# trzy/FasterRCNN

Measured on AMD Instinct MI355X. Metric: images/sec (600x1000) Faster-RCNN VGG-16 inference, higher is better.
Workload: dtype f32 (float32 tensors and accumulation; 15 GEMM layers in the f32x3 split-operand emulation = two fp16 terms per block-scaled operand, three fp16 MFMAs per product; 0 in f32x6 = three bf16 terms, six bf16 MFMAs; the other 2 on exact-f32 MFMA; strict exact-f32 everywhere: config.strict_f32_images_per_

## Files before the change

fasterrcnn_amd/_native.py:

```python
import ctypes as C
import os

_HERE = os.path.dirname(os.path.abspath(__file__))
LIB_PATH = os.environ.get("FRCNN_LIB_PATH") or os.path.join(_HERE, "csrc", "libfrcnn_hip.so")

OK = 0
ABI_VERSION = 21
ERRORS = {0: "FRCNN_OK", -1: "FRCNN_EINVAL", -2: "FRCNN_EHIP", -3: "FRCNN_ENOMEM",
          -4: "FRCNN_EUNSUPPORTED", -5: "FRCNN_ENODEVICE"}
RELU = 1
POOL2 = 2
NUM_KCLASS = 11
KCLASS_NAMES = ("conv3x3_mfma", "conv3x3_c3", "linear_mfma", "proposals", "roi_pool", "other", "winograd_transforms",
                "winograd_gemm", "winograd_x6_transforms", "winograd_x6_gemm", "winograd_x3f")

SYMBOLS = (
    "frcnn_abi_version", "frcnn_error_string", "frcnn_last_hip_error", "frcnn_device_count",
    "frcnn_anchors", "frcnn_pack_conv3x3", "frcnn_pack_conv3x3_c3", "frcnn_pack_fc_chw_to_hwc",
    "frcnn_pack_stack_rows", "frcnn_conv3x3_c3", "frcnn_conv3x3_c3_cmax", "frcnn_conv3x3_workspace_bytes", "frcnn_conv3x3_nhwc",
    "frcnn_maxpool2x2_nhwc",
    "frcnn_linear_workspace_bytes", "frcnn_linear", "frcnn_softmax_rows", "frcnn_rpn_proposals",
    "frcnn_nms", "frcnn_roi_pool", "frcnn_roi_pool_x3t", "frcnn_detections", "frcnn_ctx_create", "frcnn_ctx_create_proposals", "frcnn_ctx_destroy",
    "frcnn_ctx_bytes", "frcnn_vgg16_forward", "frcnn_ctx_tensor", "frcnn_ctx_timing_enable",
    "frcnn_ctx_timing_read",
    "frcnn_output_block_layout", "frcnn_stream_depend", "frcnn_ctx_submit_stats", "frcnn_predict_submit", "frcnn_streams_share_queue",
    "frcnn_fold_bn_pack", "frcnn_conv_workspace_bytes", "frcnn_conv_nhwc", "frcnn_conv_nhwc_math", "frcnn_conv_nhwc_x3g", "frcnn_conv_nhwc_x3g_tickets", "frcnn_pack_conv_x3g_weights", "frcnn_x3_saturation_events", "frcnn_tensor_absmax", "frcnn_conv7x7_s2_c3",
    "frcnn_maxpool3x3_s2_nhwc", "frcnn_spatial_mean_nhwc", "frcnn_resnet_forward", "frcnn_rpn_targets",
    "frcnn_preprocess_workspace_bytes", "frcnn_preprocess",
    "frcnn_conv3x3_uses_winograd", "frcnn_resnet_block_uses_winograd", "frcnn_pack_conv3x3_winograd",
    "frcnn_pack_conv3x3_winograd_taps", "frcnn_conv3x3_winograd_workspace_bytes",
    "frcnn_conv3x3_nhwc_winograd",
    "frcnn_conv3x3_uses_winograd_fused", "frcnn_resnet_block_uses_winograd_fused", "frcnn_pack_conv3x3_winograd_fused", "frcnn_pack_conv3x3_winograd_fused_taps",
    "frcnn_conv3x3_nhwc_winograd_fused",
    "frcnn_roi_align", "frcnn_roi_align_backward",
    "frcnn_x6t_record_bytes", "frcnn_split_rows_x6t", "frcnn_gemm_x6t_workspace_bytes", "frcnn_gemm_x6t", "frcnn_split_pixels_x6t", "frcnn_split_patches3x3_x6t",
    "frcnn_conv3x3_uses_winograd_x6", "frcnn_conv3x3_winograd_x6_pack_bytes", "frcnn_pack_conv3x3_winograd_x6",
    "frcnn_conv3x3_winograd_x6_workspace_bytes", "frcnn_conv3x3_nhwc_winograd_x6",
    "frcnn_pixel_absmax", "frcnn_split_pixels_x3t", "frcnn_split_patches3x3_x3t",
    "frcnn_x3t_blob_bytes", "frcnn_pack_rows_x3t", "frcnn_conv3x3_winograd_x3_pack_bytes", "frcnn_pack_conv3x3_winograd_x3",
    "frcnn_conv3x3_winograd_x3_workspace_bytes", "frcnn_conv3x3_nhwc_winograd_x3",
    "frcnn_conv3x3_winograd_x3_fused_workspace_bytes", "frcnn_conv3x3_nhwc_winograd_x3_fused", "frcnn_conv3x3_nhwc_winograd_x3_chain",
    "frcnn_x3t_record_bytes", "frcnn_rows_scale_x3t", "frcnn_split_rows_x3t", "frcnn_gemm_x3t_workspace_bytes", "frcnn_gemm_x3t",
    "frcnn_conv3x3_nhwc_winograd_fused_maps", "frcnn_ctx_create_backbone", "frcnn_resnet_backbone", "frcnn_resnet_forward_features", "frcnn_resnet_rpn_roipool", "frcnn_ctx_create_head", "frcnn_resnet_head",
    "frcnn_label_proposals", "frcnn_gather_rows", "frcnn_rpn_loss", "frcnn_detector_loss",
    "frcnn_gemm_tn_math", "frcnn_conv3x3_wgrad_math", "frcnn_conv_wgrad_math", "frcnn_bottleneck_backward_workspace_bytes", "frcnn_bottleneck_backward",
    "frcnn_gemm_tn_workspace_bytes", "frcnn_gemm_tn", "frcnn_conv3x3_wgrad_workspace_bytes", "frcnn_conv3x3_wgrad",
    "frcnn_pack_conv3x3_dgrad", "frcnn_relu_backward", "frcnn_dropout", "frcnn_dropout_relu_backward", "frcnn_add_inplace", "frcnn_maxpool2x2_backward",
    "frcnn_roi_pool_backward_workspace_bytes", "frcnn_roi_pool_backward", "frcnn_transpose", "frcnn_sgd_step", "frcnn_sgd_step_fold",
    "frcnn_conv_wgrad_workspace_bytes", "frcnn_conv_wgrad", "frcnn_conv_dgrad_workspace_bytes", "frcnn_conv_dgrad", "frcnn_conv_dgrad_math",
    "frcnn_pack_conv_dgrad", "frcnn_scale_rows", "frcnn_bn_scale_shift", "frcnn_spatial_mean_backward",
    "frcnn_ops_roi_align", "frcnn_ops_roi_align_backward", "frcnn_ops_roi_pool", "frcnn_ops_roi_pool_backward",
    "frcnn_ops_nms_workspace_bytes", "frcnn_ops_nms",
    "frcnn_ops_ms_roi_align", "frcnn_ops_ms_roi_align_workspace_bytes", "frcnn_ops_ms_roi_align_backward",
    "frcnn_ops_half_run", "frcnn_ops_roi_align_16", "frcnn_ops_roi_align_backward_16", "frcnn_ops_roi_pool_16",
    "frcnn_ops_roi_pool_backward_16", "frcnn_ops_ms_roi_align_16", "frcnn_ops_ms_roi_align_backward_16",
    "frcnn_ops_ps_roi_pool", "frcnn_ops_ps_roi_pool_backward", "frcnn_ops_ps_roi_align", "frcnn_ops_ps_roi_align_backward",
    "frcnn_ops_ps_roi_pool_16", "frcnn_ops_ps_roi_pool_backward_16", "frcnn_ops_ps_roi_align_16", "frcnn_ops_ps_roi_align_backward_16",
    "frcnn_ops_deform_workspace_bytes", "frcnn_ops_deform_forward", "frcnn_ops_deform_backward_columns", "frcnn_ops_deform_backward_offset",
    "frcnn_ops_deform_input_plan", "frcnn_ops_deform_backward_input", "frcnn_ops_deform_backward_weight",
    "frcnn_ops_deform_workspace_bytes_16", "frcnn_ops_deform_forward_16", "frcnn_ops_deform_backward_columns_16",
    "frcnn_ops_deform_backward_offset_16", "frcnn_ops_deform_input_plan_16", "frcnn_ops_deform_backward_input_16",
    "frcnn_ops_deform_backward_weight_16",
    "frcnn_ops_deform_roi_pool_cull_list", "frcnn_ops_deform_roi_pool_workspace_bytes", "frcnn_ops_deform_roi_pool",
    "frcnn_ops_deform_roi_pool_backward", "frcnn_ops_deform_roi_pool_16", "frcnn_ops_deform_roi_pool_backward_16",
    "frcnn_ops_box_iou_rotated", "frcnn_ops_nms_rotated", "frcnn_ops_roi_align_rotated_cull_list", "frcnn_ops_roi_align_rotated",
# ... 349 lines not shown
    "frcnn_maxpool3x3_s2_nhwc": (C.c_int, [_vp, _vp, _i, _i, _i, _vp]),
    "frcnn_spatial_mean_nhwc": (C.c_int, [_vp, _vp, _i, _i, _i, _i, _vp]),
    "frcnn_resnet_forward": (C.c_int, [_vp, C.POINTER(ResNetWeights), C.POINTER(ForwardParams), _vp, _i, _i,
                                       _vp, _vp, _vp, _vp, _vp, _vp, _vp]),
    "frcnn_resnet_forward_features": (C.c_int, [_vp, C.POINTER(ResNetWeights), C.POINTER(ForwardParams), _vp, _i, _i,
                                                _vp, _vp, _vp, _vp, _vp, _vp, _vp]),
    "frcnn_resnet_backbone": (C.c_int, [_vp, C.POINTER(ResNetWeights), C.POINTER(ForwardParams), _vp, _i, _i, _i, _vp, _vp]),
    "frcnn_pixel_absmax": (C.c_int, [_vp, _vp, C.c_longlong, _i, _vp]),
    "frcnn_split_pixels_x3t": (C.c_int, [_vp, _vp, _vp, _vp, _i, _i, _i, _i, _i, _i, _vp]),
    "frcnn_split_patches3x3_x3t": (C.c_int, [_vp, _vp, _vp, _vp, _i, _i, _i, _i, _i, _i, _vp]),
    "frcnn_x3t_blob_bytes": (C.c_size_t, [_i, _i, _i]),
    "frcnn_pack_rows_x3t": (C.c_int, [_vp, _i, _sz, _vp, _i, _i, _i, _i, _vp]),
    "frcnn_conv3x3_winograd_x3_pack_bytes": (C.c_size_t, [_i, _i]),
    "frcnn_pack_conv3x3_winograd_x3": (C.c_int, [_vp, _vp, _i, _i, _vp]),
    "frcnn_conv3x3_winograd_x3_workspace_bytes": (C.c_size_t, [_i, _i, _i, _i, _i]),
    "frcnn_conv3x3_nhwc_winograd_x3": (C.c_int, [_vp, _vp, _vp, _vp, _i, _i, _i, _i, _i, _u, _vp, _sz, _vp]),
    "frcnn_conv3x3_winograd_x3_fused_workspace_bytes": (C.c_size_t, [_i, _i, _i]),
    "frcnn_conv3x3_nhwc_winograd_x3_fused": (C.c_int, [_vp, _vp, _vp, _vp, _i, _i, _i, _i, _i, _u, _vp, _sz, _vp]),
    "frcnn_conv3x3_nhwc_winograd_x3_chain": (C.c_int, [_vp, _vp, _vp, _vp, _i, _i, _i, _i, _i, _u, _i, _vp, _sz, _vp, _vp, _vp]),
    "frcnn_x3t_record_bytes": (C.c_size_t, [_i, _i]),
    "frcnn_rows_scale_x3t": (C.c_int, [_vp, _i, _sz, _vp, _i, _i, _i, _i, _vp]),
    "frcnn_split_rows_x3t": (C.c_int, [_vp, _i, _sz, _vp, _vp, _i, _i, _i, _i, _vp]),
    "frcnn_gemm_x3t_workspace_bytes": (C.c_size_t, [_i, _i, _i, _i]),
    "frcnn_gemm_x3t": (C.c_int, [_vp, _vp, _i, _sz, _sz, _vp, _vp, _i, _sz, _sz, _vp, _vp, _vp, _i, _sz, _i, _i, _i, _i, _u, _vp, _sz, _vp]),
    "frcnn_ctx_create_backbone": (C.c_int, [C.POINTER(C.c_void_p), _i, _i, _i]),
    "frcnn_ctx_create_head": (C.c_int, [C.POINTER(C.c_void_p), _i]),
    "frcnn_resnet_rpn_roipool": (C.c_int, [_vp, C.POINTER(ResNetWeights), C.POINTER(ForwardParams), _vp, _i, _i, _vp, _vp, _vp, _vp, _vp, _vp]),
    "frcnn_resnet_head": (C.c_int, [_vp, C.POINTER(ResNetWeights), C.POINTER(ForwardParams), _vp, _i, _vp, _vp, _vp]),
    "frcnn_conv3x3_nhwc_winograd_fused_maps": (C.c_int, [_vp, _vp, _vp, _vp, _i, _i, _i, _i, _i, _u, _vp]),
    "frcnn_label_proposals": (C.c_int, [_vp, _vp, _i, _vp, _vp, _i, _i, _f, _f, C.POINTER(C.c_float), C.POINTER(C.c_float),
                                        _vp, _vp, _vp, _vp, _vp, _vp]),
    "frcnn_gather_rows": (C.c_int, [_vp, _vp, _i, _i, _vp, _vp]),
    "frcnn_rpn_loss": (C.c_int, [_vp, _i, _i, _vp, _i, _vp, _vp, _vp, _vp]),
    "frcnn_detector_loss": (C.c_int, [_vp, _vp, _vp, _vp, _i, _i, _vp, _vp, _i, _vp]),
    "frcnn_gemm_tn_workspace_bytes": (C.c_size_t, [_i, _i, _i]),
    "frcnn_gemm_tn": (C.c_int, [_vp, _i, _vp, _i, _vp, _i, _i, _i, _i, _vp, _sz, _vp]),
    "frcnn_gemm_tn_math": (C.c_int, [_vp, _i, _vp, _i, _vp, _i, _i, _i, _i, _i, _vp, _sz, _vp]),
    "frcnn_conv3x3_wgrad_math": (C.c_int, [_vp, _vp, _vp, _i, _i, _i, _i, _i, _vp, _sz, _vp]),
    "frcnn_conv_wgrad_math": (C.c_int, [_vp, _vp, _vp, _i, _i, _i, _i, _i, _i, _i, _i, _i, _vp, _sz, _vp]),
    "frcnn_bottleneck_backward_workspace_bytes": (C.c_int, [_vp, _vp, _vp, _vp, _i, _i, _i, _i, _i, C.POINTER(C.c_size_t), C.POINTER(C.c_size_t)]),
    "frcnn_bottleneck_backward": (C.c_int, [_vp, _vp, _vp, _vp, _vp, _vp, _vp, _vp, _vp, _vp, _vp, _vp, _vp, _i, _i, _i, _i, _i, _i, _vp, _sz, _vp, _sz,
                                            _vp, _vp]),
    "frcnn_conv3x3_wgrad_workspace_bytes": (C.c_size_t, [_i, _i, _i, _i]),
    "frcnn_conv3x3_wgrad": (C.c_int, [_vp, _vp, _vp, _i, _i, _i, _i, _vp, _sz, _vp]),
    "frcnn_pack_conv3x3_dgrad": (C.c_int, [_vp, _vp, _i, _i, _vp]),
    "frcnn_conv_wgrad_workspace_bytes": (C.c_size_t, [_i] * 8),
# ... 96 lines not shown
```

fasterrcnn_amd/csrc/api.hip:

```cpp
#include "common.h"
#include <algorithm>
#include <cmath>
#include <cstring>
#include <initializer_list>
#include <string>
#include <vector>
#include <new>

namespace frcnn {

static thread_local std::string g_hip_error;
void set_hip_error(hipError_t e) { g_hip_error = hipGetErrorString(e); }

static size_t align_up(size_t v, size_t a) { return (v + a - 1) / a * a; }

struct EventRec { int cls; hipEvent_t start, stop; };

struct Scratch {
    void* p = nullptr;
    size_t bytes = 0;
    int reserve(size_t want, hipStream_t s, bool zero)
    {
        if (want <= bytes) return FRCNN_OK;
        if (p) { FRCNN_HIP_TRY(hipStreamSynchronize(s)); release(); }
// ... 308 lines not shown
    if (!d_a || !d_inv_scale) return FRCNN_EINVAL;
    return launch_rows_scale_x3t(d_a, lda, a_batch_floats, d_inv_scale, rows, rows_padded, K, batches, as_stream(stream));
}

int frcnn_split_rows_x3t(const float* d_a, int lda, size_t a_batch_floats, const float* d_inv_scale, void* d_rec, int rows, int rows_padded,
                         int K, int batches, void* stream)
{
    if (!d_a || !d_rec || !d_inv_scale) return FRCNN_EINVAL;
    return launch_split_rows_x3t(d_a, lda, a_batch_floats, d_inv_scale, d_rec, rows, rows_padded, K, batches, as_stream(stream));
}

size_t frcnn_gemm_x3t_workspace_bytes(int M, int N, int K, int batches) { return gemm_x3t_workspace_bytes(M, N, K, batches); }

int frcnn_gemm_x3t(const void* d_a_rec, const float* d_a_inv, int a_rows, size_t a_batch_bytes, size_t a_inv_batch_floats,
                   const void* d_b_rec, const float* d_b_inv, int b_rows, size_t b_batch_bytes, size_t b_inv_batch_floats,
                   const float* d_bias, const float* d_residual, float* d_c, int ldc, size_t c_batch_floats, int M, int N, int K,
                   int batches, unsigned flags, void* d_ws, size_t ws_bytes, void* stream)
{
    return launch_gemm_x3t(d_a_rec, d_a_inv, a_rows, a_batch_bytes, a_inv_batch_floats, d_b_rec, d_b_inv, b_rows, b_batch_bytes,
                           b_inv_batch_floats, d_bias, d_residual, d_c, ldc, c_batch_floats, M, N, K, batches, flags, d_ws, ws_bytes,
                           as_stream(stream));
}

size_t frcnn_conv3x3_winograd_x3_fused_workspace_bytes(int n_maps, int H, int W)
{
    return n_maps > 0 && H > 0 && W > 0 ? conv3x3_winograd_x3_fused_workspace_bytes(n_maps, H, W) : 0;
}

int frcnn_conv3x3_nhwc_winograd_x3_fused(const float* d_x, const void* d_blob, const float* d_bias, float* d_y, int n_maps, int H, int W,
                                         int cin, int cout, unsigned flags, void* d_ws, size_t ws_bytes, void* stream)
{
    if (!d_x || !d_blob || !d_bias || !d_y) return FRCNN_EINVAL;
    return launch_conv3x3_winograd_x3_fused(d_x, d_blob, d_bias, d_y, n_maps, H, W, cin, cout, flags, d_ws, ws_bytes, as_stream(stream));
}

int frcnn_pixel_absmax(const float* d_x, float* d_cmax, long long pixels, int c, void* stream)
{
    if (!d_x || !d_cmax) return FRCNN_EINVAL;
    return launch_pixel_absmax(d_x, d_cmax, pixels, c, as_stream(stream));
}

int frcnn_split_pixels_x3t(const float* d_x, const float* d_cmax, void* d_rec, float* d_inv_scale, int n_maps, int H, int W, int c, int stride,
                           int rows_padded, void* stream)
{
    if (!d_x || !d_rec) return FRCNN_EINVAL;
    return launch_split_pixels_x3t(d_x, d_cmax, d_rec, d_inv_scale, n_maps, H, W, c, stride, rows_padded, as_stream(stream));
// ... 1582 lines not shown
```

fasterrcnn_amd/csrc/common.h:

```cpp
#pragma once
#include <hip/hip_runtime.h>
#include <stdint.h>
#include <stddef.h>
#include <stdlib.h>
#include "../../include/frcnn_hip.h"

typedef float f32x4  __attribute__((ext_vector_type(4)));
typedef float f32x16 __attribute__((ext_vector_type(16)));

inline const char* frcnn_knob(const char* name)
{
#ifdef FRCNN_EXPERIMENT_KNOBS
    return getenv(name);
#else
    (void)name;
    return nullptr;
#endif
}

namespace frcnn {

void set_hip_error(hipError_t e);

inline int check_launch() {
// ... 108 lines not shown
size_t gemm_x6t_workspace_bytes(int M, int N, int K, int batches);
void gemm_x6t_set_tiles(int mode);
int launch_gemm_x6t(const void* a_rec, int a_rows, size_t a_batch_bytes, const void* b_rec, int b_rows, size_t b_batch_bytes,
                    const float* bias, const float* residual, float* c, int ldc, size_t c_batch_floats, int M, int N, int K, int batches,
                    unsigned flags, void* ws, size_t ws_bytes, hipStream_t s, int tiles_mode = -1);
int launch_split_pixels_x6t(const float* x, void* rec, int N, int H, int W, int C, int stride, int rows_padded, hipStream_t s);
int gemm_x6t_get_tiles();
int launch_gemm_x6t_reduce(const float* ws, const float* bias, const float* residual, float* c, int ldc, size_t c_batch_floats, int M, int N,
                           int batches, int splits, int relu, hipStream_t s);
size_t x3t_record_bytes(int rows_padded, int K);
int launch_rows_scale_x3t(const float* a, int lda, size_t a_batch_floats, float* inv_scale, int R, int rows_padded, int K, int batches,
                          hipStream_t s);
int launch_split_rows_x3t(const float* a, int lda, size_t a_batch_floats, const float* inv_scale, void* rec, int R, int rows_padded, int K,
                          int batches, hipStream_t s);
int launch_split_pixels_x3t(const float* x, const float* cmax, void* rec, float* inv, int N, int H, int W, int C, int stride, int rows_padded,
                            hipStream_t s);
int launch_split_patches3x3_x3t(const float* x, const float* cmax, void* rec, float* inv, int N, int H, int W, int C, int stride,
                                int rows_padded, hipStream_t s);
size_t gemm_x3t_workspace_bytes(int M, int N, int K, int batches);
int launch_gemm_x3t(const void* a_rec, const float* a_inv, int a_rows, size_t a_batch_bytes, size_t a_inv_batch, const void* b_rec,
                    const float* b_inv, int b_rows, size_t b_batch_bytes, size_t b_inv_batch, const float* bias, const float* residual,
                    float* c, int ldc, size_t c_batch_floats, int M, int N, int K, int batches, unsigned flags, void* ws, size_t ws_bytes,
                    hipStream_t s, int tiles_mode = -1);
size_t x3t_blob_bytes(int rows_padded, int K, int batches);
int launch_pack_rows_x3t(const float* a, int lda, size_t a_batch_floats, void* blob, int R, int rows_padded, int K, int batches, hipStream_t s);
int launch_pixel_absmax(const float* x, float* cmax, long long pixels, int C, hipStream_t s);
size_t conv3x3_winograd_x3_pack_bytes(int cout, int cin);
int launch_pack_conv3x3_winograd_x3(const float* u_f32, void* ublob, int cout, int cin, hipStream_t s);
size_t conv3x3_winograd_x3_workspace_bytes(int N, int H, int W, int cin, int cout);
int winograd_x3_plan(int N, int H, int W, int cin, int cout, unsigned flags, void* ws, size_t ws_bytes, void** V, float** vinv, float** cmax,
                     float** M, void** G, size_t* g_bytes);
int launch_winograd_x3_input(const float* x, float* cmax, void* vrec, float* vinv, int N, int H, int W, int cin, hipStream_t s,
                             const float* cmax_ready = nullptr);
int launch_winograd_x3_gemm(const void* vrec, const float* vinv, const void* ublob, float* M, int N, int H, int W, int cin, int cout, void* gws,
                            size_t gws_bytes, hipStream_t s);
int launch_conv3x3_winograd_x3(const float* x, const void* ublob, const float* b, float* y, int N, int H, int W, int cin, int cout,
                               unsigned flags, void* ws, size_t ws_bytes, hipStream_t s,
                               const float* cmax_ready = nullptr, float* cmax_out = nullptr);
size_t conv3x3_winograd_x3_fused_workspace_bytes(int N, int H, int W);
int launch_conv3x3_winograd_x3_fused(const float* x, const void* ublob, const float* b, float* y, int N, int H, int W, int cin, int cout,
                                     unsigned flags, void* ws, size_t ws_bytes, hipStream_t s, const float* cmax_ready = nullptr,
                                     float* cmax_out = nullptr);
int launch_roi_pool_x3t(const float* fm, int fh, int fw, int c, const float* rois, const int32_t* n_rois, int max_rois, int pooled,
                        float scale, float* cmax, float* inv, void* rec, int rec_rows, hipStream_t s, bool cmax_ready = false);
bool conv3x3_uses_winograd_x6(int cin, int cout);
size_t conv3x3_winograd_x6_pack_bytes(int cout, int cin);
// ... 105 lines not shown
```

fasterrcnn_amd/csrc/gemm_x3t.hip:

```cpp
#include "x3t.h"

namespace frcnn {

typedef _Float16 hx_f16x8 __attribute__((ext_vector_type(8)));

#ifndef HX_ABLATE
#define HX_ABLATE 0
#endif
__global__ __launch_bounds__(256)
void rows_scale_x3t_kernel(const float* __restrict__ a, int lda, size_t a_batch, float* __restrict__ inv_scale, int R, int rows_padded,
                           int K, int batches)
{
    const int lane = threadIdx.x & 63;
    const long long wave = (long long)blockIdx.x * 4 + (threadIdx.x >> 6);
    if (wave >= (long long)batches * rows_padded) return;
    const int row = (int)(wave % rows_padded), batch = (int)(wave / rows_padded);
    float mx = 0.f;
    if (row < R) {
        const float* src = a + (size_t)batch * a_batch + (size_t)row * lda;
        for (int k = 4 * lane; k < K; k += 256) {
            const f32x4 v = *reinterpret_cast<const f32x4*>(src + k);
            mx = fmaxf(fmaxf(mx, fmaxf(fabsf(v[0]), fabsf(v[1]))), fmaxf(fabsf(v[2]), fabsf(v[3])));
        }
    }
#pragma unroll
    for (int off = 32; off >= 1; off >>= 1) mx = fmaxf(mx, __shfl_xor(mx, off));
    float mult, inv;
    hx_row_scale(mx, mult, inv);
// ... 361 lines not shown
                for (int e = 0; e < 4; ++e) v[e] = (acc[i][j][4 * g + e] * sa) * sb[e];
                if (direct && p.bias != nullptr) v = v + *reinterpret_cast<const f32x4*>(p.bias + n);
                if (direct && p.residual != nullptr)
                    v = v + *reinterpret_cast<const f32x4*>(p.residual + (size_t)batch * p.c_batch + (size_t)m * ldd + n);
                if (direct && p.relu) {
#pragma unroll
                    for (int e = 0; e < 4; ++e) v[e] = fmaxf(v[e], 0.f);
                }
                if (HX_ABLATE & 4) asm volatile("" ::"v"(v));
                else *reinterpret_cast<f32x4*>(row + n) = v;
            }
        }
    }
#ifdef HX_CLOCKS
    if (lane == 0 && p.ws != nullptr) {
        const unsigned long long real_exit = __builtin_amdgcn_s_memrealtime();
        float* o = p.ws + ((size_t)blockIdx.x * C::NW + wave) * 8;
        o[0] = (float)(clk1 - clk0); o[1] = (float)(real1 - real0); o[2] = (float)(real0 - real_entry); o[3] = (float)(real_exit - real1);
        o[4] = (float)nst; o[5] = (float)(real_entry & 0xFFFFFF); o[6] = (float)(real_exit & 0xFFFFFF); o[7] = 1.0f;
    }
#endif
}

size_t x3t_record_bytes(int rows_padded, int K) { return (size_t)(K / 16) * (rows_padded / 32) * HX_RB; }

int launch_rows_scale_x3t(const float* a, int lda, size_t a_batch_floats, float* inv_scale, int R, int rows_padded, int K, int batches,
                          hipStream_t s)
{
    if (R < 1 || rows_padded < R || rows_padded % 32 != 0 || K < 16 || K % 16 != 0 || lda < K || lda % 4 != 0 || batches < 1)
        return FRCNN_EINVAL;
    const long long waves = (long long)batches * rows_padded;
    const long long blocks = (waves + 3) / 4;
    if (blocks > 0x7fffffffLL) return FRCNN_EINVAL;
    hipLaunchKernelGGL(rows_scale_x3t_kernel, dim3((unsigned)blocks), dim3(256), 0, s, a, lda, a_batch_floats, inv_scale, R, rows_padded, K,
                       batches);
    return check_launch();
}

int launch_split_rows_x3t(const float* a, int lda, size_t a_batch_floats, const float* inv_scale, void* rec, int R, int rows_padded, int K,
                          int batches, hipStream_t s)
{
    if (R < 1 || rows_padded < R || rows_padded % 32 != 0 || K < 16 || K % 16 != 0 || lda < K || lda % 4 != 0 || batches < 1 || !inv_scale)
        return FRCNN_EINVAL;
    const long long waves = (long long)batches * (K / 16) * (rows_padded / 32);
    const long long blocks = (waves + 3) / 4;
    if (blocks > 0x7fffffffLL) return FRCNN_EINVAL;
// ... 15 lines not shown
        return check_launch();
    }
    const long long waves = (long long)(C / 16) * (rows_padded / 32);
    hipLaunchKernelGGL(split_pixels_x3t_kernel, dim3((unsigned)((waves + 3) / 4)), dim3(256), 0, s, x, cmax, static_cast<unsigned char*>(rec),
                       inv, H, W, Ho, Wo, C, stride, (int)R, rows_padded / 32, C / 16);
    return check_launch();
}

int launch_split_patches3x3_x3t(const float* x, const float* cmax, void* rec, float* inv, int N, int H, int W, int C, int stride,
                                int rows_padded, hipStream_t s)
{
    if (N < 1 || H < 1 || W < 1 || C < 16 || C % 16 != 0 || stride < 1 || stride > 2 || rows_padded % 32 != 0 || !cmax || !inv) return FRCNN_EINVAL;
    const int Ho = (H - 1) / stride + 1, Wo = (W - 1) / stride + 1;
    const long long R = (long long)N * Ho * Wo;
    if (R > rows_padded || R > 0x7fffffffLL) return FRCNN_EINVAL;
    const long long waves = (long long)(9 * C / 16) * (rows_padded / 32);
    hipLaunchKernelGGL(split_patches3x3_x3t_kernel, dim3((unsigned)((waves + 3) / 4)), dim3(256), 0, s, x, cmax,
                       static_cast<unsigned char*>(rec), inv, H, W, Ho, Wo, C, stride, (int)R, rows_padded / 32, 9 * C / 16);
    return check_launch();
}

struct HxPlan { int cfg, mtiles, ntiles, splits, chunks_per_split; };

static HxPlan plan_gemm_x3t(int M, int N, int K, int batches, int tiles_mode = -1)
{
    HxPlan pl;
    const int chunks = K / 16;
    static const int env_force = []() { const char* e = frcnn_knob("FRCNN_HX_CFG"); return e ? atoi(e) : -1; }();
    const int mode = tiles_mode >= 0 ? tiles_mode : gemm_x6t_get_tiles();
    const int force = (env_force >= 0 && tiles_mode < 0) ? env_force : (mode == 1 ? 0 : mode == 2 ? 1 : -1);
    const long long u0 = (long long)cdiv(M, 320) * cdiv(N, 256) * batches;
    const long long u1 = (long long)cdiv(M, 160) * cdiv(N, 128) * batches;
    int splits0 = 1;
    while (u0 * splits0 * 2 <= 256 && chunks / (splits0 * 2) >= 8) splits0 *= 2;
    const double c0 = (double)((u0 * splits0 + 255) / 256) * 1920.0 / splits0 + (splits0 > 1 ? 600.0 : 0.0);
    int splits1 = 1;
    while (u1 * splits1 * 2 <= 256 && chunks / (splits1 * 2) >= 8) splits1 *= 2;
    const double c1 = (double)((u1 * splits1 + 255) / 256) * 480.0 / 0.85 / splits1 + (splits1 > 1 ? 600.0 : 0.0);
    pl.cfg = (force == 0 || force == 1) ? force : (c1 < c0 ? 1 : 0);
    static const bool big_unsplit = frcnn_knob("FRCNN_HX_BIG_UNSPLIT") != nullptr;
    if (big_unsplit && force < 0 && pl.cfg == 1 && splits1 == 1) { pl.cfg = 0; splits0 = 1; }
    int splits = pl.cfg == 1 ? splits1 : splits0;
    if (splits > chunks) splits = chunks;
    pl.mtiles = pl.cfg == 1 ? cdiv(M, 160) : cdiv(M, 320);
    pl.ntiles = pl.cfg == 1 ? cdiv(N, 128) : cdiv(N, 256);
    pl.chunks_per_split = cdiv(chunks, splits);
    pl.splits = cdiv(chunks, pl.chunks_per_split);
    return pl;
}

size_t gemm_x3t_workspace_bytes(int M, int N, int K, int batches)
{
    if (!gemm_x6t_shape_ok(M, N, K, batches)) return 0;
    size_t need = 0;
    for (int mode = 0; mode < 3; ++mode) {
        const HxPlan pl = plan_gemm_x3t(M, N, K, batches, mode);
        const size_t b = pl.splits > 1 ? (size_t)pl.splits * batches * M * N * sizeof(float) : 0;
        if (b > need) need = b;
    }
    return need;
}

int launch_gemm_x3t(const void* a_rec, const float* a_inv, int a_rows, size_t a_batch_bytes, size_t a_inv_batch, const void* b_rec,
                    const float* b_inv, int b_rows, size_t b_batch_bytes, size_t b_inv_batch, const float* bias, const float* residual,
                    float* c, int ldc, size_t c_batch_floats, int M, int N, int K, int batches, unsigned flags, void* ws, size_t ws_bytes,
                    hipStream_t s, int tiles_mode)
{
    if (!gemm_x6t_shape_ok(M, N, K, batches)) return FRCNN_EUNSUPPORTED;
    if (!a_rec || !b_rec || !a_inv || !b_inv || !c || a_rows % 320 != 0 || a_rows < M || b_rows % 256 != 0 || b_rows < N || ldc < N ||
        ldc % 4 != 0)
        return FRCNN_EINVAL;
    const HxPlan pl = plan_gemm_x3t(M, N, K, batches, tiles_mode);
    if (pl.splits > 1 && (ws == nullptr || ws_bytes < (size_t)pl.splits * batches * M * N * sizeof(float))) return FRCNN_EINVAL;
    HxParams p;
    p.a = static_cast<const unsigned char*>(a_rec);
    p.b = static_cast<const unsigned char*>(b_rec);
    p.a_inv = a_inv; p.b_inv = b_inv;
    p.c = c;
    p.ws = static_cast<float*>(ws);
    p.bias = bias;
    p.residual = residual;
    p.a_batch = a_batch_bytes; p.b_batch = b_batch_bytes; p.c_batch = c_batch_floats;
    p.a_inv_batch = a_inv_batch; p.b_inv_batch = b_inv_batch;
    p.a_rbt = a_rows / 32; p.b_rbt = b_rows / 32;
    p.M = M; p.N = N; p.ldc = ldc;
    p.nchunks = K / 16; p.chunks_per_split = pl.chunks_per_split; p.splits = pl.splits; p.batches = batches;
    p.mtiles = pl.mtiles; p.ntiles = pl.ntiles;
    p.relu = (flags & FRCNN_RELU) ? 1 : 0;
    const long long total = (long long)pl.mtiles * pl.ntiles * batches * pl.splits;
    if (total > 0x7fffffffLL) return FRCNN_EINVAL;
    p.total = (int)total;
    static const int env_nsub = []() { const char* e = frcnn_knob("FRCNN_HX_NSUB"); return e ? atoi(e) : 0; }();
    const int last = p.nchunks - (pl.splits - 1) * pl.chunks_per_split;
    const bool even = pl.chunks_per_split % 2 == 0 && last % 2 == 0;
    const int nsub = !even ? 1 : (env_nsub == 1 || env_nsub == 2) ? env_nsub : (pl.chunks_per_split >= 64 ? 2 : 1);
#define HX_LAUNCH(TM, TN, VM, VN, NS)                                                                          \
    do {                                                                                                      \
        using C = HxCfg<TM, TN, VM, VN, NS>;                                                                    \
        auto kern = gemm_x3t_kernel<TM, TN, VM, VN, NS>;                                                        \
        FRCNN_MAX_LDS_ONCE(kern, C::LDS_BYTES);                                                                 \
        hipLaunchKernelGGL(kern, dim3((unsigned)total), dim3(C::THREADS), C::LDS_BYTES, s, p);                  \
    } while (0)
    if (pl.cfg == 1) { if (nsub == 2) HX_LAUNCH(5, 1, 1, 4, 2); else HX_LAUNCH(5, 1, 1, 4, 1); }
    else             { if (nsub == 2) HX_LAUNCH(5, 2, 2, 4, 2); else HX_LAUNCH(5, 2, 2, 4, 1); }
#undef HX_LAUNCH
    int rc = check_launch();
    if (rc || pl.splits == 1) return rc;
    return launch_gemm_x6t_reduce(static_cast<const float*>(ws), bias, residual, c, ldc, c_batch_floats, M, N, batches, pl.splits, p.relu, s);
}

}
```

include/frcnn_hip.h:

```cpp
#ifndef FRCNN_HIP_H
#define FRCNN_HIP_H

#include <stddef.h>
#include <stdint.h>

#ifdef __cplusplus
extern "C" {
#endif

#define FRCNN_OK            0
#define FRCNN_EINVAL       -1
#define FRCNN_EHIP         -2
#define FRCNN_ENOMEM       -3
#define FRCNN_EUNSUPPORTED -4
#define FRCNN_ENODEVICE    -5

#define FRCNN_ABI_VERSION 21

#define FRCNN_RELU   1u
#define FRCNN_POOL2  2u
#define FRCNN_X3G_WSPLIT 0x800u

int         frcnn_abi_version(void);
const char* frcnn_error_string(int code);
// ... 64 lines not shown
int frcnn_pack_rows_x3t(const float* d_a, int lda, size_t a_batch_floats, void* d_blob, int rows, int rows_padded, int K, int batches,
                        void* stream);
size_t frcnn_conv3x3_winograd_x3_pack_bytes(int cout, int cin);
int frcnn_pack_conv3x3_winograd_x3(const float* d_u_f32, void* d_blob, int cout, int cin, void* stream);
size_t frcnn_conv3x3_winograd_x3_workspace_bytes(int n_maps, int H, int W, int cin, int cout);
int frcnn_conv3x3_nhwc_winograd_x3(const float* d_x, const void* d_blob, const float* d_bias, float* d_y, int n_maps, int H, int W, int cin,
                                   int cout, unsigned flags, void* d_ws, size_t ws_bytes, void* stream);
size_t frcnn_conv3x3_winograd_x3_fused_workspace_bytes(int n_maps, int H, int W);
int frcnn_conv3x3_nhwc_winograd_x3_fused(const float* d_x, const void* d_blob, const float* d_bias, float* d_y, int n_maps, int H, int W,
                                         int cin, int cout, unsigned flags, void* d_ws, size_t ws_bytes, void* stream);
int frcnn_conv3x3_nhwc_winograd_x3_chain(const float* d_x, const void* d_blob, const float* d_bias, float* d_y, int n_maps, int H, int W, int cin,
                                         int cout, unsigned flags, int one_launch, void* d_ws, size_t ws_bytes, const float* d_cmax_in,
                                         float* d_cmax_out, void* stream);
size_t frcnn_x3t_record_bytes(int rows_padded, int K);
int frcnn_rows_scale_x3t(const float* d_a, int lda, size_t a_batch_floats, float* d_inv_scale, int rows, int rows_padded, int K, int batches,
                         void* stream);
int frcnn_split_rows_x3t(const float* d_a, int lda, size_t a_batch_floats, const float* d_inv_scale, void* d_rec, int rows, int rows_padded,
                         int K, int batches, void* stream);
size_t frcnn_gemm_x3t_workspace_bytes(int M, int N, int K, int batches);
int frcnn_gemm_x3t(const void* d_a_rec, const float* d_a_inv, int a_rows, size_t a_batch_bytes, size_t a_inv_batch_floats,
                   const void* d_b_rec, const float* d_b_inv, int b_rows, size_t b_batch_bytes, size_t b_inv_batch_floats,
                   const float* d_bias, const float* d_residual, float* d_c, int ldc, size_t c_batch_floats, int M, int N, int K,
                   int batches, unsigned flags, void* d_ws, size_t ws_bytes, void* stream);

int frcnn_split_pixels_x6t(const float* d_x, void* d_rec, int N, int H, int W, int C, int stride, int rows_padded, void* stream);
int frcnn_conv3x3_uses_winograd_x6(int cin, int cout);
size_t frcnn_conv3x3_winograd_x6_pack_bytes(int cout, int cin);
int frcnn_pack_conv3x3_winograd_x6(const float* d_w_oihw, const float* d_row_scale, void* d_u_rec, int cout, int cin, void* stream);
size_t frcnn_conv3x3_winograd_x6_workspace_bytes(int n_maps, int H, int W, int cin, int cout);
int frcnn_conv3x3_nhwc_winograd_x6(const float* d_x, const void* d_u_rec, const float* d_bias, float* d_y, int n_maps, int H, int W, int cin,
                                   int cout, unsigned flags, void* d_ws, size_t ws_bytes, void* stream);
int frcnn_split_patches3x3_x6t(const float* d_x, void* d_rec, int N, int H, int W, int C, int stride, int rows_padded, void* stream);
int frcnn_maxpool2x2_nhwc(const float* d_x, float* d_y, int H, int W, int c, void* stream);

int frcnn_fold_bn_pack(const float* d_w_oihw, const float* d_gamma, const float* d_beta,
                       const float* d_mean, const float* d_var, float eps, int cout, int cin, int ksize,
                       float* d_w_packed, float* d_b_packed, void* stream);
size_t frcnn_conv_workspace_bytes(int N, int H, int W, int cin, int cout, int ksize, int stride, int pad);
int frcnn_conv_nhwc(const float* d_x, const float* d_w_packed, const float* d_bias, const float* d_residual,
                    float* d_y, int N, int H, int W, int cin, int cout, int ksize, int stride, int pad,
                    unsigned flags, void* d_ws, size_t ws_bytes, void* stream);
int frcnn_conv7x7_s2_c3(const float* d_x_chw, const float* d_w_packed, const float* d_bias, float* d_y,
                        int H, int W, int cout, unsigned flags, void* stream);
int frcnn_maxpool3x3_s2_nhwc(const float* d_x, float* d_y, int H, int W, int c, void* stream);
int frcnn_spatial_mean_nhwc(const float* d_x, float* d_y, int N, int H, int W, int c, void* stream);

// ... 565 lines not shown
```

Measured before the change: 984.0.

## Add register-prefetched B-operand variant of the x3 split-fp16 GEMM kernel

Adds a new x3t GEMM kernel that streams only the A operand through a triple-buffered LDS pipeline. The B operand's hi/lo fp16 terms are loaded straight into registers one or two chunks ahead, and the loads are interleaved with the three MFMA terms through sched_group_barrier hints. The goal is to cut LDS traffic and barrier stalls on the B side and to hide global load latency behind MFMA work. By default it runs for the cfg-0 plan when chunks allow two sub-chunks per stage. In exchange it uses more VGPRs for the B register sets, which may lower occupancy, and it adds runtime form and big-tile knobs.

Measured after the change: 990.6 (median of 6 runs). About the same (+0.7%).

```diff
diff --git a/fasterrcnn_amd/_native.py b/fasterrcnn_amd/_native.py
--- a/fasterrcnn_amd/_native.py
+++ b/fasterrcnn_amd/_native.py
@@ -41,6 +41,7 @@
     "frcnn_conv3x3_winograd_x3_workspace_bytes", "frcnn_conv3x3_nhwc_winograd_x3",
     "frcnn_conv3x3_winograd_x3_fused_workspace_bytes", "frcnn_conv3x3_nhwc_winograd_x3_fused", "frcnn_conv3x3_nhwc_winograd_x3_chain",
     "frcnn_x3t_record_bytes", "frcnn_rows_scale_x3t", "frcnn_split_rows_x3t", "frcnn_gemm_x3t_workspace_bytes", "frcnn_gemm_x3t",
+    "frcnn_gemm_x3t_set_form", "frcnn_gemm_x3t_form",
     "frcnn_conv3x3_nhwc_winograd_fused_maps", "frcnn_ctx_create_backbone", "frcnn_resnet_backbone", "frcnn_resnet_forward_features", "frcnn_resnet_rpn_roipool", "frcnn_ctx_create_head", "frcnn_resnet_head",
     "frcnn_label_proposals", "frcnn_gather_rows", "frcnn_rpn_loss", "frcnn_detector_loss",
     "frcnn_gemm_tn_math", "frcnn_conv3x3_wgrad_math", "frcnn_conv_wgrad_math", "frcnn_bottleneck_backward_workspace_bytes", "frcnn_bottleneck_backward",
@@ -436,6 +437,8 @@
     "frcnn_rows_scale_x3t": (C.c_int, [_vp, _i, _sz, _vp, _i, _i, _i, _i, _vp]),
     "frcnn_split_rows_x3t": (C.c_int, [_vp, _i, _sz, _vp, _vp, _i, _i, _i, _i, _vp]),
     "frcnn_gemm_x3t_workspace_bytes": (C.c_size_t, [_i, _i, _i, _i]),
+    "frcnn_gemm_x3t_set_form": (C.c_int, [_i, _i]),
+    "frcnn_gemm_x3t_form": (C.c_int, [_i, _i, _i, _i]),
     "frcnn_gemm_x3t": (C.c_int, [_vp, _vp, _i, _sz, _sz, _vp, _vp, _i, _sz, _sz, _vp, _vp, _vp, _i, _sz, _i, _i, _i, _i, _u, _vp, _sz, _vp]),
     "frcnn_ctx_create_backbone": (C.c_int, [C.POINTER(C.c_void_p), _i, _i, _i]),
     "frcnn_ctx_create_head": (C.c_int, [C.POINTER(C.c_void_p), _i]),
diff --git a/fasterrcnn_amd/csrc/api.hip b/fasterrcnn_amd/csrc/api.hip
--- a/fasterrcnn_amd/csrc/api.hip
+++ b/fasterrcnn_amd/csrc/api.hip
@@ -354,6 +354,9 @@
                            as_stream(stream));
 }
 
+int frcnn_gemm_x3t_set_form(int form, int big_tiles) { return gemm_x3t_set_form(form, big_tiles); }
+int frcnn_gemm_x3t_form(int M, int N, int K, int batches) { return gemm_x3t_form(M, N, K, batches); }
+
 size_t frcnn_conv3x3_winograd_x3_fused_workspace_bytes(int n_maps, int H, int W)
 {
     return n_maps > 0 && H > 0 && W > 0 ? conv3x3_winograd_x3_fused_workspace_bytes(n_maps, H, W) : 0;
diff --git a/fasterrcnn_amd/csrc/common.h b/fasterrcnn_amd/csrc/common.h
--- a/fasterrcnn_amd/csrc/common.h
+++ b/fasterrcnn_amd/csrc/common.h
@@ -154,6 +154,8 @@
                     const float* b_inv, int b_rows, size_t b_batch_bytes, size_t b_inv_batch, const float* bias, const float* residual,
                     float* c, int ldc, size_t c_batch_floats, int M, int N, int K, int batches, unsigned flags, void* ws, size_t ws_bytes,
                     hipStream_t s, int tiles_mode = -1);
+int gemm_x3t_set_form(int form, int big_tiles);
+int gemm_x3t_form(int M, int N, int K, int batches);
 size_t x3t_blob_bytes(int rows_padded, int K, int batches);
 int launch_pack_rows_x3t(const float* a, int lda, size_t a_batch_floats, void* blob, int R, int rows_padded, int K, int batches, hipStream_t s);
 int launch_pixel_absmax(const float* x, float* cmax, long long pixels, int C, hipStream_t s);
diff --git a/fasterrcnn_amd/csrc/gemm_x3t.hip b/fasterrcnn_amd/csrc/gemm_x3t.hip
--- a/fasterrcnn_amd/csrc/gemm_x3t.hip
+++ b/fasterrcnn_amd/csrc/gemm_x3t.hip
@@ -1,9 +1,17 @@
+#include <atomic>
+
 #include "x3t.h"
 
 namespace frcnn {
 
 typedef _Float16 hx_f16x8 __attribute__((ext_vector_type(8)));
 
+#ifndef HX_BREG_AHEAD
+#define HX_BREG_AHEAD 1
+#endif
+#ifndef HX_BREG_DEFAULT
+#define HX_BREG_DEFAULT 1
+#endif
 #ifndef HX_ABLATE
 #define HX_ABLATE 0
 #endif
@@ -411,6 +419,219 @@
 #endif
 }
 
+template <int V> struct HxInt { static constexpr int value = V; };
+
+template <class C, int WTM, int WTN>
+__device__ __forceinline__ void hx_epilogue(const HxParams& p, f32x16 (&acc)[WTM][WTN], int batch, int split, int mt, int nt, int wm, int wn, int lane)
+{
+    const bool direct = p.splits == 1;
+    float* dst;
+    int ldd;
+    if (direct) { dst = p.c + (size_t)batch * p.c_batch; ldd = p.ldc; }
+    else        { dst = p.ws + ((size_t)split * p.batches + batch) * (size_t)p.M * p.N; ldd = p.N; }
+    const int m_base = mt * C::BM + 32 * WTM * wm + (lane & 31);
+    const int n_base = nt * C::BN + 32 * WTN * wn + 4 * (lane >> 5);
+    const float* ainv = p.a_inv + (size_t)batch * p.a_inv_batch;
+    const float* binv = p.b_inv + (size_t)batch * p.b_inv_batch;
+#pragma unroll
+    for (int i = 0; i < WTM; ++i) {
+        const int m = m_base + 32 * i;
+        if (m >= p.M) continue;
+        const float sa = ainv[m];
+        float* row = dst + (size_t)m * ldd;
+#pragma unroll
+        for (int j = 0; j < WTN; ++j) {
+#pragma unroll
+            for (int g = 0; g < 4; ++g) {
+                const int n = n_base + 32 * j + 8 * g;
+                if (n >= p.N) continue;
+                const f32x4 sb = *reinterpret_cast<const f32x4*>(binv + n);
+                f32x4 v;
+#pragma unroll
+                for (int e = 0; e < 4; ++e) v[e] = (acc[i][j][4 * g + e] * sa) * sb[e];
+                if (direct && p.bias != nullptr) v = v + *reinterpret_cast<const f32x4*>(p.bias + n);
+                if (direct && p.residual != nullptr)
+                    v = v + *reinterpret_cast<const f32x4*>(p.residual + (size_t)batch * p.c_batch + (size_t)m * ldd + n);
+                if (direct && p.relu) {
+#pragma unroll
+                    for (int e = 0; e < 4; ++e) v[e] = fmaxf(v[e], 0.f);
+                }
+                if (HX_ABLATE & 4) asm volatile("" ::"v"(v));
+                else *reinterpret_cast<f32x4*>(row + n) = v;
+            }
+        }
+    }
+}
+
+template <int WTM, int WTN, int WVM, int WVN, int NSUB, int BD>
+struct HxRegCfg {
+    using T = HxCfg<WTM, WTN, WVM, WVN, NSUB>;
+    static constexpr int NW = T::NW, THREADS = T::THREADS, BM = T::BM, BN = T::BN, BRB = T::BRB;
+    static constexpr int A_BYTES = T::A_BYTES;
+    static constexpr int STAGE = NSUB * A_BYTES;
+    static constexpr int NBUF = 3, DIST = 2;
+    static constexpr size_t LDS_BYTES = NBUF * (size_t)STAGE;
+    static constexpr int PPW = (NSUB * T::NPA + NW - 1) / NW;
+    static constexpr int NB = 2 * WTN;
+    static constexpr int NSETS = BD + 1;
+    static constexpr int PERIOD = NSETS % NSUB == 0 ? NSETS / NSUB : NSETS;
+    static_assert(BD >= 1 && BD <= NSUB && NSETS <= 3 && NSUB <= 2, "register sets: one or two chunks ahead, at most a stage");
+    static_assert(WTM * WTN >= PPW + WTN, "the lo x hi product covers the DMA pieces and the early register loads");
+};
+
+template <int WTM, int WTN, int WVM, int WVN, int NSUB, int BD>
+__global__ __launch_bounds__(64 * WVM * WVN, 2)
+void gemm_x3t_breg_kernel(const HxParams p)
+{
+    using C = HxRegCfg<WTM, WTN, WVM, WVN, NSUB, BD>;
+    extern __shared__ __attribute__((aligned(16))) unsigned char smem_hx[];
+    const int tid = threadIdx.x, lane = tid & 63;
+    const int wave = __builtin_amdgcn_readfirstlane(tid >> 6);
+    const int wm = wave / WVN, wn = wave % WVN;
+
+    int bid = blockIdx.x;
+    {
+        const int q = p.total >> 3, r = p.total & 7, xcd = bid & 7, idx = bid >> 3;
+        bid = (xcd < r ? xcd * (q + 1) : r * (q + 1) + (xcd - r) * q) + idx;
+    }
+    const int nt = bid % p.ntiles;
+    int t = bid / p.ntiles;
+    const int mt = t % p.mtiles;
+    t /= p.mtiles;
+    const int split = t % p.splits;
+    const int batch = t / p.splits;
+
+    const int c_begin = split * p.chunks_per_split;
+    int c_end = c_begin + p.chunks_per_split;
+    if (c_end > p.nchunks) c_end = p.nchunks;
+    const int nch = c_end - c_begin;
+    const int nst = nch / NSUB;
+
+    const int a_chunk = p.a_rbt * HX_RB, b_chunk = p.b_rbt * HX_RB;
+    const __amdgpu_buffer_rsrc_t ars = __builtin_amdgcn_make_buffer_rsrc(const_cast<unsigned char*>(p.a + (size_t)batch * p.a_batch), 0, p.nchunks * a_chunk, 0x00020000);
+    const __amdgpu_buffer_rsrc_t brs = __builtin_amdgcn_make_buffer_rsrc(const_cast<unsigned char*>(p.b + (size_t)batch * p.b_batch), 0, p.nchunks * b_chunk, 0x00020000);
+    const int a_base = mt * C::A_BYTES + c_begin * a_chunk;
+    const int b_base = (nt * C::BRB + wn * WTN) * HX_RB + c_begin * b_chunk;
+    const int lane16 = lane * 16;
+
+    auto issue_a = [&](int s, int buf) {
+        const int as = a_base + s * NSUB * a_chunk;
+        unsigned char* ldsb = smem_hx + buf * C::STAGE;
+#pragma unroll
+        for (int i = 0; i < C::PPW; ++i) {
+            int q = wave + C::NW * i;
+            q = q < NSUB * C::T::NPA ? q : NSUB * C::T::NPA - 1;
+            const int sub = q / C::T::NPA, r = q - sub * C::T::NPA;
+            __builtin_amdgcn_raw_ptr_buffer_load_lds(ars, (hx_lds_ptr)(ldsb + sub * C::A_BYTES + r * HX_PIECE), 16, lane16, as + sub * a_chunk + r * HX_PIECE, 0, 0);
+        }
+    };
+    f32x16 acc[WTM][WTN];
+#pragma unroll
+    for (int i = 0; i < WTM; ++i)
+#pragma unroll
+        for (int j = 0; j < WTN; ++j)
+#pragma unroll
+            for (int r = 0; r < 16; ++r) acc[i][j][r] = 0.f;
+
+    hx_f16x8 ah[WTM], al[WTM], bh[C::NSETS][WTN], bl[C::NSETS][WTN];
+#pragma unroll
+    for (int i = 0; i < WTM; ++i)
+#pragma unroll
+        for (int e = 0; e < 8; ++e) al[i][e] = (_Float16)0.f;
+#pragma unroll
+    for (int j = 0; j < WTN; ++j)
+#pragma unroll
+        for (int e = 0; e < 8; ++e) bh[BD][j][e] = (_Float16)0.f;
+
+    auto load_bl = [&](int c, auto SET) {
+        const int so = b_base + (c < nch ? c : nch - 1) * b_chunk;
+#pragma unroll
+        for (int j = 0; j < WTN; ++j)
+            bl[decltype(SET)::value][j] = __builtin_bit_cast(hx_f16x8, __builtin_amdgcn_raw_buffer_load_b128(brs, lane16 + j * HX_RB + HX_PIECE, so, 0));
+    };
+    auto load_bh = [&](int c, auto SET) {
+        const int so = b_base + (c < nch ? c : nch - 1) * b_chunk;
+#pragma unroll
+        for (int j = 0; j < WTN; ++j)
+            bh[decltype(SET)::value][j] = __builtin_bit_cast(hx_f16x8, __builtin_amdgcn_raw_buffer_load_b128(brs, lane16 + j * HX_RB, so, 0));
+    };
+
+#define HX_SGB(mask, n) __builtin_amdgcn_sched_group_barrier(mask, n, 0)
+#define HX_TERM(A, B)                                                                                  \
+    _Pragma("unroll") for (int i = 0; i < WTM; ++i)                                                     \
+        _Pragma("unroll") for (int j = 0; j < WTN; ++j)                                                 \
+            acc[i][j] = __builtin_amdgcn_mfma_f32_32x32x16_f16(B[j], A[i], acc[i][j], 0, 0, 0);
+
+    if (nst > 0) {
+        load_bl(0, HxInt<0>{}); load_bh(0, HxInt<0>{});
+        if constexpr (BD == 2) { load_bl(1, HxInt<1>{}); load_bh(1, HxInt<1>{}); }
+        issue_a(0, 0);
+        issue_a(nst > 1 ? 1 : 0, 1);
+        asm volatile("s_waitcnt vmcnt(%0)" ::"n"(C::PPW) : "memory");
+        __builtin_amdgcn_s_barrier();
+        int cur = 0;
+        const int a_off = wm * WTM * HX_RB + lane * 16;
+
+        auto chunk = [&](int s, int nxt, auto SUB, auto SET) {
+            constexpr int sub = decltype(SUB)::value, set = decltype(SET)::value, pset = (set + C::NSETS - 1) % C::NSETS;
+            const unsigned char* at = smem_hx + cur * C::STAGE + sub * C::A_BYTES + a_off;
+#pragma unroll
+            for (int i = 0; i < WTM; ++i) ah[i] = *reinterpret_cast<const hx_f16x8*>(at + i * HX_RB);
+            if constexpr (sub == 0) issue_a(s + C::DIST < nst ? s + C::DIST : nst - 1, nxt);
+            load_bl(s * NSUB + sub + BD, HxInt<pset>{});
+            HX_TERM(al, bh[pset])
+            load_bh(s * NSUB + sub + BD, HxInt<pset>{});
+            HX_TERM(ah, bl[set])
+#pragma unroll
+            for (int i = 0; i < WTM; ++i) al[i] = *reinterpret_cast<const hx_f16x8*>(at + i * HX_RB + HX_PIECE);
+            HX_TERM(ah, bh[set])
+#if !HX_NO_SCHED
+            constexpr int NT = WTM * WTN, PW = sub == 0 ? C::PPW : 0;
+            HX_SGB(0x100, WTM);
+            _Pragma("unroll") for (int q = 0; q < PW + WTN; ++q) { HX_SGB(0x008, 1); HX_SGB(0x010, 1); }
+            HX_SGB(0x008, NT - PW - WTN);
+            HX_SGB(0x010, WTN);
+            _Pragma("unroll") for (int q = 0; q < (WTM < NT ? WTM : NT); ++q) { HX_SGB(0x008, 1); HX_SGB(0x100, 1); }
+            if (NT > WTM) HX_SGB(0x008, NT - WTM);
+            HX_SGB(0x008, NT);
+#endif
+        };
+        auto stage = [&](int s, auto K) {
+            constexpr int ph = (decltype(K)::value * NSUB) % C::NSETS;
+            const int nxt = cur == 0 ? 2 : cur - 1;
+            chunk(s, nxt, HxInt<0>{}, HxInt<ph>{});
+            if constexpr (NSUB == 2) chunk(s, nxt, HxInt<1>{}, HxInt<(ph + 1) % C::NSETS>{});
+            __builtin_amdgcn_sched_barrier(0);
+            asm volatile("s_waitcnt vmcnt(%0) lgkmcnt(0)" ::"n"(C::PPW + NSUB * C::NB) : "memory");
+            __builtin_amdgcn_s_barrier();
+            cur = cur == C::NBUF - 1 ? 0 : cur + 1;
+            __builtin_amdgcn_sched_barrier(0);
+        };
+        int s = 0;
+        for (; s + C::PERIOD <= nst; s += C::PERIOD) {
+            stage(s, HxInt<0>{});
+            if constexpr (C::PERIOD > 1) stage(s + 1, HxInt<1>{});
+            if constexpr (C::PERIOD > 2) stage(s + 2, HxInt<2>{});
+        }
+        if constexpr (C::PERIOD > 1) { if (s < nst) { stage(s, HxInt<0>{}); ++s; } }
+        if constexpr (C::PERIOD > 2) { if (s < nst) { stage(s, HxInt<1>{}); ++s; } }
+        const int ls = (nch - 1) % C::NSETS;
+        hx_f16x8 bt[WTN];
+#pragma unroll
+        for (int j = 0; j < WTN; ++j) {
+            bt[j] = bh[C::NSETS - 1][j];
+#pragma unroll
+            for (int q = 0; q < C::NSETS - 1; ++q) bt[j] = ls == q ? bh[q][j] : bt[j];
+        }
+        HX_TERM(al, bt)
+        asm volatile("s_waitcnt vmcnt(0)" ::: "memory");
+    }
+#undef HX_TERM
+#undef HX_SGB
+
+    hx_epilogue<C, WTM, WTN>(p, acc, batch, split, mt, nt, wm, wn, (int)__builtin_amdgcn_mbcnt_hi(~0u, __builtin_amdgcn_mbcnt_lo(~0u, 0u)));
+}
+
 size_t x3t_record_bytes(int rows_padded, int K) { return (size_t)(K / 16) * (rows_padded / 32) * HX_RB; }
 
 int launch_rows_scale_x3t(const float* a, int lda, size_t a_batch_floats, float* inv_scale, int R, int rows_padded, int K, int batches,
@@ -472,11 +693,22 @@
 
 struct HxPlan { int cfg, mtiles, ntiles, splits, chunks_per_split; };
 
+static std::atomic<int> g_hx_form{0}, g_hx_big_tiles{0};
+
+int gemm_x3t_set_form(int form, int big_tiles)
+{
+    if (form < 0 || form > 2) return FRCNN_EINVAL;
+    g_hx_form.store(form);
+    g_hx_big_tiles.store(big_tiles ? 1 : 0);
+    return FRCNN_OK;
+}
+
 static HxPlan plan_gemm_x3t(int M, int N, int K, int batches, int tiles_mode = -1)
 {
     HxPlan pl;
     const int chunks = K / 16;
     static const int env_force = []() { const char* e = frcnn_knob("FRCNN_HX_CFG"); return e ? atoi(e) : -1; }();
+    if (tiles_mode < 0 && g_hx_big_tiles.load()) tiles_mode = 1;
     const int mode = tiles_mode >= 0 ? tiles_mode : gemm_x6t_get_tiles();
     const int force = (env_force >= 0 && tiles_mode < 0) ? env_force : (mode == 1 ? 0 : mode == 2 ? 1 : -1);
     const long long u0 = (long long)cdiv(M, 320) * cdiv(N, 256) * batches;
@@ -497,6 +729,28 @@
     pl.chunks_per_split = cdiv(chunks, splits);
     pl.splits = cdiv(chunks, pl.chunks_per_split);
     return pl;
+}
+
+static int hx_nsub(const HxPlan& pl, int nchunks, int env_nsub, bool* even_out)
+{
+    const int last = nchunks - (pl.splits - 1) * pl.chunks_per_split;
+    const bool even = pl.chunks_per_split % 2 == 0 && last % 2 == 0;
+    if (even_out) *even_out = even;
+    return !even ? 1 : (env_nsub == 1 || env_nsub == 2) ? env_nsub : (pl.chunks_per_split >= 64 ? 2 : 1);
+}
+
+static bool hx_takes_breg(const HxPlan& pl, int nsub, int a_rows, int b_rows, int K)
+{
+    const int form = g_hx_form.load();
+    const bool fits = (long long)K * a_rows < (1LL << 29) && (long long)K * b_rows < (1LL << 29);
+    return pl.cfg == 0 && fits && (form == 2 || (form == 0 && HX_BREG_DEFAULT && nsub == 2));
+}
+
+int gemm_x3t_form(int M, int N, int K, int batches)
+{
+    if (!gemm_x6t_shape_ok(M, N, K, batches)) return FRCNN_EUNSUPPORTED;
+    const HxPlan pl = plan_gemm_x3t(M, N, K, batches);
+    return hx_takes_breg(pl, hx_nsub(pl, K / 16, 0, nullptr), cdiv(M, 320) * 320, cdiv(N, 256) * 256, K) ? 1 : 0;
 }
 
 size_t gemm_x3t_workspace_bytes(int M, int N, int K, int batches)
@@ -541,9 +795,19 @@
     if (total > 0x7fffffffLL) return FRCNN_EINVAL;
     p.total = (int)total;
     static const int env_nsub = []() { const char* e = frcnn_knob("FRCNN_HX_NSUB"); return e ? atoi(e) : 0; }();
-    const int last = p.nchunks - (pl.splits - 1) * pl.chunks_per_split;
-    const bool even = pl.chunks_per_split % 2 == 0 && last % 2 == 0;
-    const int nsub = !even ? 1 : (env_nsub == 1 || env_nsub == 2) ? env_nsub : (pl.chunks_per_split >= 64 ? 2 : 1);
+    bool even;
+    const int nsub = hx_nsub(pl, p.nchunks, env_nsub, &even);
+    if (hx_takes_breg(pl, nsub, a_rows, b_rows, K)) {
+#define HX_LAUNCH_BREG(NS, BD)                                                                                 \
+    do {                                                                                                      \
+        using C = HxRegCfg<5, 2, 2, 4, NS, BD>;                                                                 \
+        auto kern = gemm_x3t_breg_kernel<5, 2, 2, 4, NS, BD>;                                                   \
+        FRCNN_MAX_LDS_ONCE(kern, C::LDS_BYTES);                                                                 \
+        hipLaunchKernelGGL(kern, dim3((unsigned)total), dim3(C::THREADS), C::LDS_BYTES, s, p);                  \
+    } while (0)
+        if (even) HX_LAUNCH_BREG(2, HX_BREG_AHEAD); else HX_LAUNCH_BREG(1, 1);
+#undef HX_LAUNCH_BREG
+    } else {
 #define HX_LAUNCH(TM, TN, VM, VN, NS)                                                                          \
     do {                                                                                                      \
         using C = HxCfg<TM, TN, VM, VN, NS>;                                                                    \
@@ -554,6 +818,7 @@
     if (pl.cfg == 1) { if (nsub == 2) HX_LAUNCH(5, 1, 1, 4, 2); else HX_LAUNCH(5, 1, 1, 4, 1); }
     else             { if (nsub == 2) HX_LAUNCH(5, 2, 2, 4, 2); else HX_LAUNCH(5, 2, 2, 4, 1); }
 #undef HX_LAUNCH
+    }
     int rc = check_launch();
     if (rc || pl.splits == 1) return rc;
     return launch_gemm_x6t_reduce(static_cast<const float*>(ws), bias, residual, c, ldc, c_batch_floats, M, N, batches, pl.splits, p.relu, s);
diff --git a/include/frcnn_hip.h b/include/frcnn_hip.h
--- a/include/frcnn_hip.h
+++ b/include/frcnn_hip.h
@@ -110,6 +110,8 @@
                    const void* d_b_rec, const float* d_b_inv, int b_rows, size_t b_batch_bytes, size_t b_inv_batch_floats,
                    const float* d_bias, const float* d_residual, float* d_c, int ldc, size_t c_batch_floats, int M, int N, int K,
                    int batches, unsigned flags, void* d_ws, size_t ws_bytes, void* stream);
+int frcnn_gemm_x3t_set_form(int form, int big_tiles);
+int frcnn_gemm_x3t_form(int M, int N, int K, int batches);
 
 int frcnn_split_pixels_x6t(const float* d_x, void* d_rec, int N, int H, int W, int C, int stride, int rows_padded, void* stream);
 int frcnn_conv3x3_uses_winograd_x6(int cin, int cout);
```
